# anoma/taiga

Measured on NVIDIA H100. Metric: partial-tx proofs/sec, higher is better.
Workload: dtype u32x8 (255-bit Montgomery integers, Pasta Fp/Fq)

## Files before the change

### taiga_b200/csrc/msm.cu

```cuda
#include <memory>
#include "common.cuh"
#include "kernels.cuh"

namespace tb {

constexpr int MSM_CHUNK_MAX = 64;
constexpr int MSM_SEG = 8;
constexpr int MSM_FIXED_C = 13;
constexpr uint32_t MSM_HEAVY_UNITS = 1024;

int msm_default_window(int n, bool fixed_tables) {
  if (fixed_tables) return MSM_FIXED_C;
  int lg = 0; while ((1 << (lg + 1)) <= n) ++lg;
  int c = lg - 4;
  if (c < 4) c = 4;
  if (c > 16) c = 16;
  return c;
}

__device__ __forceinline__ uint32_t window_bits(const uint32_t* s, int bit, int c) {
  int limb = bit >> 5, off = bit & 31;
  uint64_t v = s[limb];
  if (limb + 1 < 8) v |= (uint64_t)s[limb + 1] << 32;
  return (uint32_t)(v >> off) & ((1u << c) - 1);
// ... 193 lines not shown
    { const uint32_t* src = reinterpret_cast<const uint32_t*>(&acc); uint32_t* dst = reinterpret_cast<uint32_t*>(&o);
#pragma unroll
      for (int i = 0; i < 32; ++i) dst[i] = __shfl_down_sync(0xffffffffu, src[i], d, 16); }
    if ((int)l < d) acc.add(o);
  }
  if (live && l == 0) lines[line] = acc;
}
template <class B>
__global__ void __launch_bounds__(256) msm_weighted_kernel(const Xyzz<B>* __restrict__ lines, int s_log, int h_log, Xyzz<B>* __restrict__ out, Aff<B>* __restrict__ aff_out) {
  extern __shared__ uint4 mw_smem[];
  Xyzz<B>* sm = reinterpret_cast<Xyzz<B>*>(mw_smem);
  const int S = 1 << s_log, H = 1 << h_log, half = blockDim.x >> 1;
  const int part = threadIdx.x >= (unsigned)half, j = threadIdx.x - part * half, len = part ? H : S;
  const Xyzz<B>* src = lines + (size_t)blockIdx.x * (S + H) + (part ? S : 0);
  Xyzz<B>* v = sm + part * half;
  Xyzz<B> acc = j < len ? src[j] : Xyzz<B>::inf();
  v[j] = acc;
  __syncthreads();
  for (int d = 1; d < half; d <<= 1) {
    const bool act = j + d < len;
    Xyzz<B> o;
    if (act) o = v[j + d];
    __syncthreads();
    if (act) { acc.add(o); v[j] = acc; }
    __syncthreads();
  }
  if (part && j == 0) v[0] = Xyzz<B>::inf();
  __syncthreads();
  for (int d = half >> 1; d >= 1; d >>= 1) {
    if (j < d) { Xyzz<B> a = v[j]; a.add(v[j + d]); v[j] = a; }
    __syncthreads();
  }
  if (threadIdx.x == 0) {
    Xyzz<B> r = sm[half];
    for (int i = 0; i < s_log; ++i) r = r.dbl();
    r.add(sm[0]);
    out[blockIdx.x] = r;
    if (aff_out) aff_out[blockIdx.x] = r.to_affine();
  }
}

template <class B>
__global__ void __launch_bounds__(256) msm_window_kernel(const Xyzz<B>* __restrict__ seg_out, int nt, Xyzz<B>* __restrict__ win_out) {
  __shared__ Xyzz<B> sm[8];
  uint32_t g = blockIdx.x;
  Xyzz<B> acc = Xyzz<B>::inf();
  for (int t = threadIdx.x; t < nt; t += blockDim.x) acc.add(seg_out[(size_t)g * nt + t]);
  acc = block_reduce_pt(acc, sm);
  if (threadIdx.x == 0) win_out[g] = acc;
}

template <class B>
__global__ void msm_horner_kernel(const Xyzz<B>* __restrict__ win, int wsep, int c, int K, Xyzz<B>* __restrict__ out) {
  int k = blockIdx.x * blockDim.x + threadIdx.x;
  if (k >= K) return;
  Xyzz<B> acc = win[(size_t)k * wsep + wsep - 1];
  for (int w = wsep - 2; w >= 0; --w) {
    for (int i = 0; i < c; ++i) acc = acc.dbl();
    acc.add(win[(size_t)k * wsep + w]);
  }
  out[k] = acc;
}

template <class B, class S>
void msm_run(Ctx* ctx, const S* scalars, long long scalar_bstride, const Aff<B>* bases, long long base_bstride, int N, int K,
             const MsmConfig& cfg_in, Xyzz<B>* out) {
  TB_REQUIRE(N >= 1 && K >= 1 && K <= 65535, "MSM shape out of range");
  const bool table_mode = cfg_in.table_windows > 0;
  int c = cfg_in.c ? cfg_in.c : msm_default_window(N, table_mode);
  TB_REQUIRE(c >= 2 && c <= 20, "MSM window out of range");
  const int W = (256 + c - 1) / c;
  if (table_mode) TB_REQUIRE(cfg_in.table_windows >= W, "fixed-base table has too few windows");
  const int NB = 1 << (c - 1);
  const int wsep = table_mode ? 1 : W;
  const uint64_t nb_total64 = (uint64_t)K * wsep * NB;
  const int n_extra = table_mode ? cfg_in.n_extra : 0;
  const int table_stride = table_mode ? (cfg_in.table_stride ? cfg_in.table_stride : N) : 0;
  const uint64_t max_entries = (uint64_t)K * (N + n_extra) * W;
  TB_REQUIRE(nb_total64 < (1ull << 31) && max_entries < (1ull << 32) && (uint64_t)(N + 2) * (table_mode ? W : 1) < (1ull << 31), "MSM too large");
  const uint32_t nb_total = (uint32_t)nb_total64;
  cudaStream_t st = ctx->stream;

  DevBuf<Xyzz<B>> buckets(ctx, nb_total);
  ctx->work[PC_MSM_SORT] += 2.0 * (double)K * (N + n_extra);
  ctx->work[PC_MSM_REDUCE] += (double)K * wsep * NB * 30.0;
  std::unique_ptr<ProfScope> ps;
  if (msm_batch_applicable(N, K, cfg_in, c)) {
    msm_batch_buckets<B, S>(ctx, scalars, scalar_bstride, bases, N, K, c, W, table_stride, reinterpret_cast<const S*>(cfg_in.extra_scalars), n_extra, buckets.get());
    ctx->launches -= 6;
  } else {
    DevBuf<uint32_t> counts(ctx, nb_total), offs(ctx, nb_total + 1), cursor(ctx, nb_total), entries(ctx, max_entries);
    ps.reset(new ProfScope(ctx, PC_MSM_SORT));
    counts.zero();
    dim3 dg((N + n_extra + 255) / 256, K);
    const S* extras = reinterpret_cast<const S*>(cfg_in.extra_scalars);
    msm_digits_kernel<S, 0><<<dg, 256, 0, st>>>(scalars, scalar_bstride, N, c, W, NB, wsep, table_mode, table_stride, extras, n_extra, counts.get(), nullptr);
    TB_LAUNCH_CHECK();
    exclusive_scan_u32(ctx, counts.get(), offs.get(), nb_total);
    TB_CUDA(cudaMemcpyAsync(cursor.get(), offs.get(), nb_total * sizeof(uint32_t), cudaMemcpyDeviceToDevice, st));
    msm_digits_kernel<S, 1><<<dg, 256, 0, st>>>(scalars, scalar_bstride, N, c, W, NB, wsep, table_mode, table_stride, extras, n_extra, cursor.get(), entries.get());
    TB_LAUNCH_CHECK();

    uint32_t chunk_log = 3;
    { const uint64_t target_units = (uint64_t)tb_tune("TB_MSM_UNITS_PER_SM", 2048) * (uint64_t)ctx->sm_count;
      while ((1u << chunk_log) < (uint32_t)MSM_CHUNK_MAX && (max_entries >> chunk_log) > target_units) ++chunk_log; }
    const uint64_t max_units = nb_total64 + (max_entries >> chunk_log) + 1;
    const uint64_t max_heavy = (max_entries >> chunk_log) / MSM_HEAVY_UNITS + 1;
    uint32_t lpb_log = 0;
    { const uint64_t avg_units = ((max_entries >> chunk_log) + nb_total64 - 1) / nb_total64;
      const uint64_t warps_target = (uint64_t)tb_tune("TB_MSM_SUB_WARPS_PER_SM", 16) * (uint64_t)ctx->sm_count;
      while (lpb_log < 5 && ((nb_total64 << (lpb_log + 1)) >> 5) <= warps_target && (1ull << lpb_log) < avg_units) ++lpb_log; }
    const uint32_t sub_units = 4u << lpb_log;
    uint64_t max_mid = (max_entries >> chunk_log) / sub_units + 1;
    if (max_mid > nb_total64) max_mid = nb_total64;
    DevBuf<uint32_t> unit_count(ctx, nb_total), unit_off(ctx, nb_total + 1), mid(ctx, max_mid), heavy(ctx, max_heavy), n_lists(ctx, 2);
    n_lists.zero();
    msm_units_kernel<<<(nb_total + 255) / 256, 256, 0, st>>>(offs.get(), nb_total, chunk_log, sub_units, unit_count.get(), mid.get(), heavy.get(), n_lists.get());
    TB_LAUNCH_CHECK();
    exclusive_scan_u32(ctx, unit_count.get(), unit_off.get(), nb_total);
    DevBuf<Xyzz<B>> partial(ctx, max_units);
    ctx->work[PC_MSM_ACCUM] += 10.5 * (double)max_entries * 0.97;
    ps.reset(); ps.reset(new ProfScope(ctx, PC_MSM_ACCUM));
    { const unsigned ag = (unsigned)((max_units + 127) / 128);
      const int minb = tb_tune("TB_MSM_ACCUM_MINB", 4);
      if (minb >= 6) msm_accum_kernel<B, 6><<<ag, 128, 0, st>>>(bases, base_bstride, (uint32_t)wsep * NB, offs.get(), unit_off.get(), nb_total, 1u << chunk_log, entries.get(), partial.get());
      else if (minb == 5) msm_accum_kernel<B, 5><<<ag, 128, 0, st>>>(bases, base_bstride, (uint32_t)wsep * NB, offs.get(), unit_off.get(), nb_total, 1u << chunk_log, entries.get(), partial.get());
      else msm_accum_kernel<B, 4><<<ag, 128, 0, st>>>(bases, base_bstride, (uint32_t)wsep * NB, offs.get(), unit_off.get(), nb_total, 1u << chunk_log, entries.get(), partial.get()); }
    TB_LAUNCH_CHECK();
    ps.reset(); ps.reset(new ProfScope(ctx, PC_MSM_REDUCE));
    msm_combine_sub_kernel<B><<<(unsigned)((((uint64_t)nb_total << lpb_log) + 127) / 128), 128, 0, st>>>(unit_off.get(), partial.get(), nb_total, lpb_log,
                                                                                                        buckets.get());
    { uint64_t g = (max_mid + 7) / 8, cap = 4ull * (uint64_t)ctx->sm_count;
      msm_combine_kernel<B><<<(unsigned)(g < cap ? g : cap), 256, 0, st>>>(mid.get(), n_lists.get(), unit_off.get(), partial.get(), buckets.get()); }
    if ((max_entries >> chunk_log) > MSM_HEAVY_UNITS)
      msm_combine_heavy_kernel<B><<<(unsigned)(max_heavy < 296 ? max_heavy : 296), 256, 0, st>>>(heavy.get(), n_lists.get() + 1, unit_off.get(), partial.get(), buckets.get());
    TB_LAUNCH_CHECK();
    ps.reset();
  }
  ps.reset(new ProfScope(ctx, PC_MSM_REDUCE));

  const int seg_t = tb_tune("TB_MSM_SEG", MSM_SEG);
  const int seg = NB < seg_t ? NB : seg_t;
  const int nt = NB / seg;
  const uint32_t groups = (uint32_t)K * wsep;
  Aff<B>* const aff_out = reinterpret_cast<Aff<B>*>(cfg_in.affine_out);
  if (wsep == 1 && NB < 64) {
    int threads = ((nt + 31) / 32) * 32;
    msm_bucket_reduce_kernel<B><<<groups, threads, 0, st>>>(buckets.get(), NB, seg, nt, out, aff_out);
    TB_LAUNCH_CHECK();
    ctx->launches += 6;
    return;
  }
  if (wsep == 1) {
    const int lb = c - 1, s_log = (lb + 1) / 2, h_log = lb - s_log;
    const int nl = (1 << s_log) + (1 << h_log), threads = 2 << s_log;
    TB_REQUIRE(threads <= 256, "fixed-base window too wide for the weighted-sum kernel (c <= 15)");
    DevBuf<Xyzz<B>> lines(ctx, (size_t)groups * nl);
    msm_linesum_kernel<B><<<(unsigned)(((uint64_t)groups * nl * 16 + 127) / 128), 128, 0, st>>>(buckets.get(), NB, s_log, groups, lines.get());
    TB_LAUNCH_CHECK();
    const size_t smem = (size_t)threads * sizeof(Xyzz<B>);
    if (smem > 48 * 1024) {
      ctx->opt_in_smem(msm_weighted_kernel<B>, 128 * 1024);
    }
    msm_weighted_kernel<B><<<groups, threads, smem, st>>>(lines.get(), s_log, h_log, out, aff_out);
    TB_LAUNCH_CHECK();
    ctx->launches += 7;
    return;
  }
  DevBuf<Xyzz<B>> seg_out(ctx, (size_t)groups * nt), win(ctx, groups);
  msm_segsum_kernel<B><<<(groups * nt + 127) / 128, 128, 0, st>>>(buckets.get(), NB, seg, nt, groups, seg_out.get());
  TB_LAUNCH_CHECK();
  msm_window_kernel<B><<<groups, 256, 0, st>>>(seg_out.get(), nt, win.get());
  TB_LAUNCH_CHECK();
  msm_horner_kernel<B><<<(K + 31) / 32, 32, 0, st>>>(win.get(), wsep, c, K, out);
// ... 65 lines not shown
```

### taiga_b200/csrc/msm_batch.cu

```cuda
#define TB_NOINLINE_MUL 0
#include <cuda.h>
#include <algorithm>
#include <memory>
#include <type_traits>
#include "common.cuh"
#include "kernels.cuh"

namespace tb {

constexpr int BA_THREADS = 256;
constexpr int BA_M = 32;
constexpr int BA_PAIRS = BA_THREADS * BA_M;
constexpr int BA_MAX_NB = 4096;
constexpr int SORT_THREADS = 1024;
constexpr int SORT_TILE = 1024;
constexpr int SORT_BOX = 256;

__device__ __forceinline__ void block_scan_excl(uint32_t* v, int n, uint32_t* tmp) {
  const int T = blockDim.x, t = threadIdx.x, per = (n + T - 1) / T;
  const int b0 = t * per, b1 = min(n, b0 + per);
  uint32_t local = 0;
  for (int i = b0; i < b1; ++i) local += v[i];
  uint32_t incl = local;
  const int lane = t & 31, warp = t >> 5, nw = (T + 31) >> 5;
#pragma unroll
  for (int d = 1; d < 32; d <<= 1) { uint32_t o = __shfl_up_sync(0xffffffffu, incl, d); if (lane >= d) incl += o; }
  if (lane == 31) tmp[warp] = incl;
  __syncthreads();
  if (warp == 0) {
    uint32_t w = lane < nw ? tmp[lane] : 0u, wi = w;
#pragma unroll
    for (int d = 1; d < 32; d <<= 1) { uint32_t o = __shfl_up_sync(0xffffffffu, wi, d); if (lane >= d) wi += o; }
    if (lane < nw) tmp[lane] = wi - w;
    if (lane == nw - 1) v[n] = wi;
  }
  __syncthreads();
  uint32_t run = tmp[warp] + incl - local;
  for (int i = b0; i < b1; ++i) { uint32_t x = v[i]; v[i] = run; run += x; }
  __syncthreads();
}

__device__ __forceinline__ uint32_t smem_u32(const void* p) { return (uint32_t)__cvta_generic_to_shared(p); }
__device__ __forceinline__ void mbar_init(uint64_t* bar, uint32_t count) {
  asm volatile("mbarrier.init.shared::cta.b64 [%0], %1;" ::"r"(smem_u32(bar)), "r"(count) : "memory");
}
__device__ __forceinline__ void mbar_expect_tx(uint64_t* bar, uint32_t bytes) {
  asm volatile("mbarrier.arrive.expect_tx.shared::cta.b64 _, [%0], %1;" ::"r"(smem_u32(bar)), "r"(bytes) : "memory");
}
__device__ __forceinline__ void mbar_wait(uint64_t* bar, uint32_t parity) {
  uint32_t done = 0;
  for (uint32_t spin = 0; spin < (1u << 26); ++spin) {
    asm volatile("{ .reg .pred p; mbarrier.try_wait.parity.shared::cta.b64 p, [%1], %2; selp.u32 %0, 1, 0, p; }" : "=r"(done) : "r"(smem_u32(bar)), "r"(parity) : "memory");
    if (done) return;
  }
  __trap();
}
__device__ __forceinline__ void tma_load_tile(void* dst, const CUtensorMap* map, uint64_t* bar, int scalar0, int item) {
  asm volatile("cp.async.bulk.tensor.3d.shared::cluster.global.tile.mbarrier::complete_tx::bytes [%0], [%1, {%3, %4, %5}], [%2];"
               ::"r"(smem_u32(dst)), "l"(map), "r"(smem_u32(bar)), "r"(0), "r"(scalar0), "r"(item) : "memory");
}

template <class S, int CT>
__global__ void __launch_bounds__(SORT_THREADS) msm_sort_kernel(const __grid_constant__ CUtensorMap smap, const S* __restrict__ extras, int N, int n_extra, int c_rt, int W_rt,
                                                                 int NB, int table_stride, uint32_t* __restrict__ counts, uint32_t* __restrict__ entries, long long cap0,
                                                                 unsigned long long* __restrict__ total_entries) {
  const int c = CT ? CT : c_rt, W = CT ? (256 + CT - 1) / CT : W_rt;
  extern __shared__ __align__(128) uint8_t sort_smem[];
  S* tile = reinterpret_cast<S*>(sort_smem);
  uint64_t* bars = reinterpret_cast<uint64_t*>(sort_smem + 2 * SORT_TILE * sizeof(S));
  uint32_t* hist = reinterpret_cast<uint32_t*>(bars + 2);
  uint32_t* tmp = hist + NB + 1;
  const int k = blockIdx.x, t = threadIdx.x;
  const uint32_t half = 1u << (c - 1);
  const int ntiles = (N + SORT_TILE - 1) / SORT_TILE;
  if (t == 0) { mbar_init(&bars[0], 1); mbar_init(&bars[1], 1); asm volatile("fence.mbarrier_init.release.cluster;" ::: "memory"); }
  for (int b = t; b <= NB; b += SORT_THREADS) hist[b] = 0;
  __syncthreads();
  uint32_t* ent = entries + (long long)k * cap0;

  auto digits = [&](const S& sm, uint32_t idx, auto scatter_c) {
    constexpr bool scatter = decltype(scatter_c)::value;
    S s = sm.from_mont();
    if (s.is_zero()) return;
    uint32_t carry = 0;
#pragma unroll
    for (int w = 0; w < W; ++w) {
      const int bit = w * c, limb = bit >> 5, off = bit & 31;
      uint64_t v64 = s.l[limb];
      if (limb + 1 < 8) v64 |= (uint64_t)s.l[limb + 1] << 32;
      uint32_t v = ((uint32_t)(v64 >> off) & ((1u << c) - 1)) + carry, neg = 0;
      if (v > half) { v = (1u << c) - v; neg = 1; carry = 1; } else carry = 0;
      if (v) {
        if (scatter) { const uint32_t pos = atomicAdd(&hist[v - 1], 1u); ent[pos] = (uint32_t)(w * table_stride + idx) | (neg << 31); }
        else atomicAdd(&hist[v - 1], 1u);
      }
    }
  };
  auto issue = [&](int stage, int it) {
    const int s0 = it * SORT_TILE;
    int nbox = (N - s0 + SORT_BOX - 1) / SORT_BOX; if (nbox > SORT_TILE / SORT_BOX) nbox = SORT_TILE / SORT_BOX;
    mbar_expect_tx(&bars[stage], (uint32_t)(nbox * SORT_BOX * sizeof(S)));
    for (int j = 0; j < nbox; ++j) tma_load_tile(tile + stage * SORT_TILE + j * SORT_BOX, &smap, &bars[stage], s0 + j * SORT_BOX, k);
  };
  uint32_t phase[2] = {0, 0};
  for (int pass = 0; pass < 2; ++pass) {
    if (t == 0) issue(0, 0);
    for (int it = 0; it < ntiles; ++it) {
      const int st = it & 1;
      if (t == 0 && it + 1 < ntiles) issue(st ^ 1, it + 1);
      mbar_wait(&bars[st], phase[st]); phase[st] ^= 1;
      const int i = it * SORT_TILE + t;
      if (i < N) { if (pass) digits(tile[st * SORT_TILE + t], (uint32_t)i, std::true_type()); else digits(tile[st * SORT_TILE + t], (uint32_t)i, std::false_type()); }
      __syncthreads();
    }
    if (t < n_extra) { const S ex = ldg_fe(extras + (long long)k * n_extra + t); if (pass) digits(ex, (uint32_t)(N + t), std::true_type()); else digits(ex, (uint32_t)(N + t), std::false_type()); }
    __syncthreads();
    if (pass == 0) {
      for (int b = t; b < NB; b += SORT_THREADS) counts[(long long)k * NB + b] = hist[b];
      __syncthreads();
      block_scan_excl(hist, NB, tmp);
      if (t == 0) atomicAdd(total_entries, (unsigned long long)hist[NB]);
    }
  }
}

template <class F> __device__ __forceinline__ void sts_fe(uint4* lo, uint4* hi, int idx, const F& v) {
  lo[idx] = make_uint4(v.l[0], v.l[1], v.l[2], v.l[3]); hi[idx] = make_uint4(v.l[4], v.l[5], v.l[6], v.l[7]);
}
template <class F> __device__ __forceinline__ F lds_fe(const uint4* lo, const uint4* hi, int idx) {
  uint4 x = lo[idx], y = hi[idx]; F v;
  v.l[0] = x.x; v.l[1] = x.y; v.l[2] = x.z; v.l[3] = x.w; v.l[4] = y.x; v.l[5] = y.y; v.l[6] = y.z; v.l[7] = y.w; return v;
}

enum { PK_NONE = 0, PK_COPY1, PK_COPY2, PK_ADD, PK_DBL, PK_INF };

struct RoundOffsets {
  uint32_t* off_cur; uint32_t* off_nxt; uint32_t n_next;
  __device__ __forceinline__ void build(uint8_t* smem, const uint32_t* __restrict__ counts0, int NB, int round) {
    off_cur = reinterpret_cast<uint32_t*>(smem); off_nxt = off_cur + (NB + 4);
    uint32_t* tmp = off_nxt + (NB + 4);
    for (int b = threadIdx.x; b < NB; b += blockDim.x) {
      const uint32_t c0 = counts0[b], cr = (c0 + ((1u << round) - 1)) >> round;
      off_cur[b] = cr; off_nxt[b] = (cr + 1) >> 1;
    }
    __syncthreads();
    block_scan_excl(off_cur, NB, tmp);
    block_scan_excl(off_nxt, NB, tmp);
    n_next = off_nxt[NB];
  }
  __device__ __forceinline__ void locate(uint32_t q, int NB, uint32_t& in0, bool& two, int& hint) const {
    int lo = hint;
#pragma unroll 1
    for (int s = 0; s < 6 && off_nxt[lo + 1] <= q; ++s) ++lo;
    if (off_nxt[lo + 1] <= q) {
      int hi = NB;
      while (hi - lo > 1) { const int mid = (lo + hi) >> 1; if (off_nxt[mid] <= q) lo = mid; else hi = mid; }
    }
    hint = lo;
    in0 = off_cur[lo] + 2 * (q - off_nxt[lo]);
    two = in0 + 1 < off_cur[lo + 1];
  }
};
constexpr size_t ba_off_bytes(int NB) { return (size_t)(2 * (NB + 4) + 32) * 4; }

template <class B, bool FIRST> struct PairLoader {
  const uint32_t* entries; const Aff<B>* table; const Aff<B>* items;
  __device__ __forceinline__ Aff<B> point(uint32_t pos) const {
    if (FIRST) {
      const uint32_t e = __ldg(entries + pos);
      Aff<B> p = ldg_aff(table + (e & 0x7fffffffu));
      if (e >> 31) p.y = p.y.neg();
      return p;
    }
    return ldg_aff(items + pos);
  }
  __device__ __forceinline__ B x(uint32_t pos) const {
    if (FIRST) return ldg_fe(&table[__ldg(entries + pos) & 0x7fffffffu].x);
    return ldg_fe(&items[pos].x);
  }
};
template <class B> __device__ __forceinline__ int classify_pair(const Aff<B>& p1, const Aff<B>& p2, bool two, B& den) {
  if (!two || p2.is_inf()) return PK_COPY1;
  if (p1.is_inf()) return PK_COPY2;
  den = p2.x - p1.x;
  if (!den.is_zero()) return PK_ADD;
  if (p1.y == p2.y && !p1.y.is_zero()) { den = p1.y.dbl(); return PK_DBL; }
  return PK_INF;
}

__global__ void __launch_bounds__(BA_THREADS) msm_ba_count_kernel(const uint32_t* __restrict__ counts0, int NB, int R, uint32_t* __restrict__ n_items) {
  __shared__ uint32_t red[BA_THREADS / 32];
  const int k = blockIdx.x, t = threadIdx.x;
  for (int r = 0; r <= R; ++r) {
    uint32_t s = 0;
    for (int b = t; b < NB; b += BA_THREADS) s += (counts0[(long long)k * NB + b] + ((1u << r) - 1)) >> r;
    for (int d = 16; d >= 1; d >>= 1) s += __shfl_down_sync(0xffffffffu, s, d);
    if ((t & 31) == 0) red[t >> 5] = s;
    __syncthreads();
    if (t == 0) { uint32_t tot = 0; for (int w = 0; w < BA_THREADS / 32; ++w) tot += red[w]; n_items[(long long)k * (R + 1) + r] = tot; }
    __syncthreads();
  }
}

template <class B, bool FIRST, int M>
__global__ void __launch_bounds__(BA_THREADS) msm_ba_fwd_kernel(const uint32_t* __restrict__ counts0, int NB, int round, const uint32_t* __restrict__ entries,
// ... 41 lines not shown
template <class B>
__global__ void msm_ba_inv_kernel(B* __restrict__ tree, uint32_t n_trees) {
  const uint32_t i = blockIdx.x * blockDim.x + threadIdx.x;
  if (i >= n_trees) return;
  B* root = tree + (size_t)i * (2 * BA_THREADS) + 1;
  st_fe(root, ld_fe(root).inv());
}

template <class B, bool FIRST, int M, int MINB>
__global__ void __launch_bounds__(BA_THREADS, MINB) msm_ba_bwd_kernel(const uint32_t* __restrict__ counts0, int NB, int round, const uint32_t* __restrict__ entries,
                                                                 const Aff<B>* __restrict__ table, const Aff<B>* __restrict__ items_in, long long cap_in,
                                                                 Aff<B>* __restrict__ items_out, long long cap_out, const B* __restrict__ pre, const B* __restrict__ tree,
                                                                 const uint32_t* __restrict__ meta, const uint32_t* __restrict__ n_items, int R) {
  extern __shared__ __align__(16) uint8_t ba_smem[];
  const int k = blockIdx.y, t = threadIdx.x;
  const uint32_t Q0 = blockIdx.x * (M * BA_THREADS);
  const uint32_t n_next = n_items[(long long)k * (R + 1) + round + 1];
  if (Q0 >= n_next) return;
  B* nd = reinterpret_cast<B*>(ba_smem);
  { const B* tr = tree + ((long long)k * gridDim.x + blockIdx.x) * (2 * BA_THREADS);
    nd[t] = ld_fe(tr + t); nd[BA_THREADS + t] = ld_fe(tr + BA_THREADS + t); }
  __syncthreads();
  for (int w = 1; w < BA_THREADS; w <<= 1) {
    B child_inv;
    const int node = w + (t >> 1);
    if (t < 2 * w) child_inv = nd[node] * nd[2 * node + ((t & 1) ^ 1)];
    __syncthreads();
    if (t < 2 * w) nd[2 * node + (t & 1)] = child_inv;
    __syncthreads();
  }
  B inv_run = nd[BA_THREADS + t];
  PairLoader<B, FIRST> ld{entries + (FIRST ? (long long)k * cap_in : 0), table, items_in + (FIRST ? 0 : (long long)k * cap_in)};
  const B* pre_k = pre + (long long)k * cap_out;
  const uint32_t* meta_k = meta + (long long)k * cap_out;
  Aff<B>* out = items_out + (long long)k * cap_out;
  int last = M - 1;
  while (last >= 0 && Q0 + (uint32_t)last * BA_THREADS + t >= n_next) --last;
#pragma unroll 1
  for (int i = last; i >= 0; --i) {
    const uint32_t q = Q0 + (uint32_t)i * BA_THREADS + t;
    const uint32_t mt = __ldg(meta_k + q);
    const uint32_t in0 = mt & 0x7fffffffu; const bool two = mt >> 31;
    const Aff<B> p1 = ld.point(in0);
    Aff<B> p2 = p1;
    if (two) p2 = ld.point(in0 + 1);
    B den;
    const int kind = classify_pair(p1, p2, two, den);
    Aff<B> r;
    if (kind == PK_COPY1) r = p1;
    else if (kind == PK_COPY2) r = p2;
    else if (kind == PK_INF) r = Aff<B>::inf();
    else {
      const B dinv = inv_run * ldg_fe(pre_k + q);
      inv_run = inv_run * den;
      B num;
      if (kind == PK_ADD) num = p2.y - p1.y;
      else { const B x2 = p1.x.sqr(); num = x2.dbl() + x2; }
      const B lam = num * dinv;
      r.x = lam.sqr() - p1.x - p2.x;
      r.y = lam * (p1.x - r.x) - p1.y;
    }
    st_fe(&out[q].x, r.x); st_fe(&out[q].y, r.y);
  }
}

template <class B>
__global__ void __launch_bounds__(BA_THREADS) msm_ba_finish_kernel(const uint32_t* __restrict__ counts0, int NB, int round, const Aff<B>* __restrict__ items, long long cap,
                                                                    Xyzz<B>* __restrict__ buckets) {
  extern __shared__ __align__(16) uint8_t fin_smem[];
  uint32_t* off = reinterpret_cast<uint32_t*>(fin_smem);
  uint32_t* tmp = off + NB + 4;
  const int k = blockIdx.y, t = threadIdx.x;
  for (int b = t; b < NB; b += BA_THREADS) { uint32_t c0 = counts0[(long long)k * NB + b]; off[b] = (c0 + ((1u << round) - 1)) >> round; }
  __syncthreads();
  block_scan_excl(off, NB, tmp);
  const int b = blockIdx.x * BA_THREADS + t;
  if (b >= NB) return;
  Xyzz<B> acc = Xyzz<B>::inf();
  const Aff<B>* it = items + (long long)k * cap;
  for (uint32_t p = off[b]; p < off[b + 1]; ++p) acc.add_affine(ldg_aff(it + p));
  buckets[(long long)k * NB + b] = acc;
}

typedef CUresult (*EncodeTiledFn)(CUtensorMap*, CUtensorMapDataType, cuuint32_t, void*, const cuuint64_t*, const cuuint64_t*, const cuuint32_t*, const cuuint32_t*,
                                  CUtensorMapInterleave, CUtensorMapSwizzle, CUtensorMapL2promotion, CUtensorMapFloatOOBfill);
static EncodeTiledFn encode_tiled_fn() {
  static EncodeTiledFn fn = nullptr;
  if (!fn) {
    void* p = nullptr; cudaDriverEntryPointQueryResult qr;
    TB_CUDA(cudaGetDriverEntryPoint("cuTensorMapEncodeTiled", &p, cudaEnableDefault, &qr));
    if (qr != cudaDriverEntryPointSuccess || !p) throw CudaError("cuTensorMapEncodeTiled is not available from this driver");
    fn = reinterpret_cast<EncodeTiledFn>(p);
  }
  return fn;
}

template <class B, bool FIRST, int M, int MINB>
static void launch_round_t(Ctx* ctx, dim3 grid, size_t fwd_smem, size_t bwd_smem, const uint32_t* counts, int NB, int r, const uint32_t* entries, const Aff<B>* table, const Aff<B>* in,
                           long long cap_in, Aff<B>* out, long long cap_out, B* pre, B* tree, uint32_t* meta, const uint32_t* n_items, int R, uint32_t n_trees) {
  cudaStream_t st = ctx->stream;
  ctx->opt_in_smem(msm_ba_fwd_kernel<B, FIRST, M>, fwd_smem);
  ctx->opt_in_smem(msm_ba_bwd_kernel<B, FIRST, M, MINB>, bwd_smem);
  msm_ba_fwd_kernel<B, FIRST, M><<<grid, BA_THREADS, fwd_smem, st>>>(counts, NB, r, entries, table, in, cap_in, cap_out, pre, tree, meta, n_items, R);
  msm_ba_inv_kernel<B><<<(n_trees + 63) / 64, 64, 0, st>>>(tree, n_trees);
  msm_ba_bwd_kernel<B, FIRST, M, MINB><<<grid, BA_THREADS, bwd_smem, st>>>(counts, NB, r, entries, table, in, cap_in, out, cap_out, pre, tree, meta, n_items, R);
}
template <class B, typename... A> static void launch_round(Ctx* ctx, int M, int minb, bool first, A... a) {
#define TB_LR(MM, NN) (first ? launch_round_t<B, true, MM, NN>(ctx, a...) : launch_round_t<B, false, MM, NN>(ctx, a...))
  if (M == 8) { if (minb == 2) TB_LR(8, 2); else if (minb == 3) TB_LR(8, 3); else TB_LR(8, 4); }
  else if (M == 32) { if (minb == 2) TB_LR(32, 2); else if (minb == 3) TB_LR(32, 3); else TB_LR(32, 4); }
  else { if (minb == 2) TB_LR(16, 2); else if (minb == 3) TB_LR(16, 3); else TB_LR(16, 4); }
#undef TB_LR
}

bool msm_batch_applicable(int N, int K, const MsmConfig& cfg, int c) {
  if (cfg.table_windows <= 0 || (1 << (c - 1)) > BA_MAX_NB || c < 6) return false;
  const long long min_terms = tb_tune("TB_MSM_BA_MIN_TERMS", 1 << 21);
  return (long long)N * K >= min_terms;
}

template <class B, class S>
void msm_batch_buckets(Ctx* ctx, const S* scalars, long long sstride, const Aff<B>* table, int N, int K, int c, int W, int table_stride, const S* extras, int n_extra,
                       Xyzz<B>* buckets) {
  const int NB = 1 << (c - 1);
  cudaStream_t st = ctx->stream;
  TB_REQUIRE(((uintptr_t)scalars & 15) == 0 && (sstride * (long long)sizeof(S)) % 16 == 0, "scalar vectors must be 16-byte aligned for TMA");
  const long long cap0 = (long long)(N + n_extra) * W;
  std::vector<long long> cap(1, cap0);
  const int R = tb_tune("TB_MSM_BA_ROUNDS", 10);
  TB_REQUIRE(R >= 1 && R <= 20, "TB_MSM_BA_ROUNDS out of range");
  for (int r = 0; r < R; ++r) cap.push_back((cap.back() + NB + 1) / 2);
  const int Kc_max = tb_tune("TB_MSM_BA_CHUNK", ctx->sm_count);
  const int Kc = K < Kc_max ? K : Kc_max;
  DevBuf<uint32_t> counts(ctx, (size_t)Kc * NB), entries(ctx, (size_t)Kc * cap0);
  DevBuf<Aff<B>> itA(ctx, (size_t)Kc * cap[1]), itB(ctx, (size_t)Kc * (R > 1 ? cap[2] : 1));
  const size_t sort_smem = 2 * SORT_TILE * sizeof(S) + 16 + (size_t)(NB + 1 + 32) * 4 + 16;
  const size_t fwd_smem = std::max(ba_off_bytes(NB), (size_t)2 * BA_THREADS * sizeof(B));
  const size_t bwd_smem = (size_t)2 * BA_THREADS * sizeof(B);
  const size_t fin_smem = (size_t)(NB + 4 + 32) * 4;
  ctx->opt_in_smem(msm_sort_kernel<S, 13>, sort_smem);
  ctx->opt_in_smem(msm_sort_kernel<S, 0>, sort_smem);
  ctx->opt_in_smem(msm_ba_finish_kernel<B>, fin_smem);
  const int Mv = tb_tune("TB_MSM_BA_M", 32) >= 32 ? 32 : tb_tune("TB_MSM_BA_M", 32) <= 8 ? 8 : 16, minb = tb_tune("TB_MSM_BA_MINB", 3) <= 2 ? 2 : tb_tune("TB_MSM_BA_MINB", 3) >= 4 ? 4 : 3;
  const long long pairs_per_cta = (long long)Mv * BA_THREADS;
  const unsigned ctas1 = (unsigned)((cap[1] + pairs_per_cta - 1) / pairs_per_cta);
  DevBuf<B> pre(ctx, (size_t)Kc * cap[1]), tree(ctx, (size_t)Kc * ctas1 * 2 * BA_THREADS);
  DevBuf<uint32_t> meta(ctx, (size_t)Kc * cap[1]), n_items(ctx, (size_t)Kc * (R + 1));
  for (int k0 = 0; k0 < K; k0 += Kc) {
    const int kc = K - k0 < Kc ? K - k0 : Kc;
    { ProfScope ps(ctx, PC_MSM_SORT);
      CUtensorMap smap;
      const cuuint64_t dims[3] = {8, (cuuint64_t)N, (cuuint64_t)kc};
      const cuuint64_t strides[2] = {sizeof(S), (cuuint64_t)sstride * sizeof(S)};
      const cuuint32_t box[3] = {8, SORT_BOX, 1}, estr[3] = {1, 1, 1};
      CUresult cr = encode_tiled_fn()(&smap, CU_TENSOR_MAP_DATA_TYPE_UINT32, 3, const_cast<S*>(scalars + (long long)k0 * sstride), dims, strides, box, estr,
                                      CU_TENSOR_MAP_INTERLEAVE_NONE, CU_TENSOR_MAP_SWIZZLE_NONE, CU_TENSOR_MAP_L2_PROMOTION_L2_128B, CU_TENSOR_MAP_FLOAT_OOB_FILL_NONE);
      if (cr != CUDA_SUCCESS) throw CudaError("cuTensorMapEncodeTiled failed for the scalar tensor (" + std::to_string((int)cr) + ")");
      const S* ex = extras ? extras + (long long)k0 * n_extra : nullptr;
      if (c == 13) msm_sort_kernel<S, 13><<<kc, SORT_THREADS, sort_smem, st>>>(smap, ex, N, extras ? n_extra : 0, c, W, NB, table_stride, counts.get(), entries.get(), cap0, ctx->d_msm_adds);
      else msm_sort_kernel<S, 0><<<kc, SORT_THREADS, sort_smem, st>>>(smap, ex, N, extras ? n_extra : 0, c, W, NB, table_stride, counts.get(), entries.get(), cap0, ctx->d_msm_adds);
      TB_LAUNCH_CHECK(); ctx->launches++; }
    { ProfScope ps(ctx, PC_MSM_ACCUM);
      msm_ba_count_kernel<<<kc, BA_THREADS, 0, st>>>(counts.get(), NB, R, n_items.get());
      for (int r = 0; r < R; ++r) {
        const Aff<B>* in = (r & 1) ? itA.get() : itB.get();
        Aff<B>* out = (r & 1) ? itB.get() : itA.get();
        const unsigned gx = (unsigned)((cap[r + 1] + pairs_per_cta - 1) / pairs_per_cta);
        dim3 grid(gx, kc);
        const uint32_t n_trees = gx * (uint32_t)kc;
        launch_round<B>(ctx, Mv, minb, r == 0, grid, fwd_smem, bwd_smem, counts.get(), NB, r, entries.get(), table, in, r == 0 ? cap0 : cap[r], out, cap[r + 1], pre.get(), tree.get(),
                        meta.get(), n_items.get(), R, n_trees);
        TB_LAUNCH_CHECK(); ctx->launches += 3;
      }
      const Aff<B>* last = (R & 1) ? itA.get() : itB.get();
      msm_ba_finish_kernel<B><<<dim3((NB + BA_THREADS - 1) / BA_THREADS, kc), BA_THREADS, fin_smem, st>>>(counts.get(), NB, R, last, cap[R], buckets + (size_t)k0 * NB);
      TB_LAUNCH_CHECK(); ctx->launches++; }
  }
}

template void msm_batch_buckets<Fq, Fp>(Ctx*, const Fp*, long long, const Aff<Fq>*, int, int, int, int, int, const Fp*, int, Xyzz<Fq>*);
template void msm_batch_buckets<Fp, Fq>(Ctx*, const Fq*, long long, const Aff<Fp>*, int, int, int, int, int, const Fq*, int, Xyzz<Fp>*);

}
```

Before: 14.93.

## Replace per-MSM single-CTA TMA bucket sort with tiled digit/prefix/scatter kernels

The old sort used one 1024-thread CTA per MSM, streaming scalars through TMA twice (a count pass and a scatter pass), so parallelism was limited to K blocks. The new path splits the scalars into tiles spread over many CTAs. A digit kernel writes packed 16-bit signed digits and per-tile histograms, a prefix kernel scans the histograms across tiles, and a scatter kernel stages entries in shared memory, then writes them out in bucket order with warp-aggregated atomics. This adds an intermediate digit buffer, extra global traffic and two more launches, and entry order within a bucket now differs.

After: 15.50, median of 6. +3.8%, better.

```diff
diff --git a/taiga_b200/csrc/msm.cu b/taiga_b200/csrc/msm.cu
--- a/taiga_b200/csrc/msm.cu
+++ b/taiga_b200/csrc/msm.cu
@@ -299,14 +299,15 @@
   cudaStream_t st = ctx->stream;
 
   DevBuf<Xyzz<B>> buckets(ctx, nb_total);
-  ctx->work[PC_MSM_SORT] += 2.0 * (double)K * (N + n_extra);
   ctx->work[PC_MSM_REDUCE] += (double)K * wsep * NB * 30.0;
   std::unique_ptr<ProfScope> ps;
   if (msm_batch_applicable(N, K, cfg_in, c)) {
+    ctx->work[PC_MSM_SORT] += (double)K * (N + n_extra);
     msm_batch_buckets<B, S>(ctx, scalars, scalar_bstride, bases, N, K, c, W, table_stride, reinterpret_cast<const S*>(cfg_in.extra_scalars), n_extra, buckets.get());
     ctx->launches -= 6;
   } else {
     DevBuf<uint32_t> counts(ctx, nb_total), offs(ctx, nb_total + 1), cursor(ctx, nb_total), entries(ctx, max_entries);
+    ctx->work[PC_MSM_SORT] += 2.0 * (double)K * (N + n_extra);
     ps.reset(new ProfScope(ctx, PC_MSM_SORT));
     counts.zero();
     dim3 dg((N + n_extra + 255) / 256, K);
diff --git a/taiga_b200/csrc/msm_batch.cu b/taiga_b200/csrc/msm_batch.cu
--- a/taiga_b200/csrc/msm_batch.cu
+++ b/taiga_b200/csrc/msm_batch.cu
@@ -1,8 +1,6 @@
 #define TB_NOINLINE_MUL 0
-#include <cuda.h>
 #include <algorithm>
 #include <memory>
-#include <type_traits>
 #include "common.cuh"
 #include "kernels.cuh"
 
@@ -12,9 +10,12 @@
 constexpr int BA_M = 32;
 constexpr int BA_PAIRS = BA_THREADS * BA_M;
 constexpr int BA_MAX_NB = 4096;
-constexpr int SORT_THREADS = 1024;
-constexpr int SORT_TILE = 1024;
-constexpr int SORT_BOX = 256;
+constexpr int DIG_THREADS = 256;
+constexpr int PREFIX_THREADS = 256;
+constexpr int SCAT_THREADS = 1024;
+constexpr int TILE_ENTRIES = 20480;
+__host__ __device__ constexpr int tile_log(int W) { return W <= 20 ? 10 : W <= 40 ? 9 : 8; }
+__host__ __device__ constexpr int dig_stride(int W) { return (W + 3) & ~3; }
 
 __device__ __forceinline__ void block_scan_excl(uint32_t* v, int n, uint32_t* tmp) {
   const int T = blockDim.x, t = threadIdx.x, per = (n + T - 1) / T;
@@ -40,87 +41,147 @@
   __syncthreads();
 }
 
-__device__ __forceinline__ uint32_t smem_u32(const void* p) { return (uint32_t)__cvta_generic_to_shared(p); }
-__device__ __forceinline__ void mbar_init(uint64_t* bar, uint32_t count) {
-  asm volatile("mbarrier.init.shared::cta.b64 [%0], %1;" ::"r"(smem_u32(bar)), "r"(count) : "memory");
-}
-__device__ __forceinline__ void mbar_expect_tx(uint64_t* bar, uint32_t bytes) {
-  asm volatile("mbarrier.arrive.expect_tx.shared::cta.b64 _, [%0], %1;" ::"r"(smem_u32(bar)), "r"(bytes) : "memory");
-}
-__device__ __forceinline__ void mbar_wait(uint64_t* bar, uint32_t parity) {
-  uint32_t done = 0;
-  for (uint32_t spin = 0; spin < (1u << 26); ++spin) {
-    asm volatile("{ .reg .pred p; mbarrier.try_wait.parity.shared::cta.b64 p, [%1], %2; selp.u32 %0, 1, 0, p; }" : "=r"(done) : "r"(smem_u32(bar)), "r"(parity) : "memory");
-    if (done) return;
-  }
-  __trap();
-}
-__device__ __forceinline__ void tma_load_tile(void* dst, const CUtensorMap* map, uint64_t* bar, int scalar0, int item) {
-  asm volatile("cp.async.bulk.tensor.3d.shared::cluster.global.tile.mbarrier::complete_tx::bytes [%0], [%1, {%3, %4, %5}], [%2];"
-               ::"r"(smem_u32(dst)), "l"(map), "r"(smem_u32(bar)), "r"(0), "r"(scalar0), "r"(item) : "memory");
-}
+template <bool RET> __device__ __forceinline__ uint32_t bucket_add(uint32_t* ctr, uint32_t key) {
+  const uint32_t ones = __ballot_sync(0xffffffffu, key == 0);
+  uint32_t slot = 0;
+  if (ones) {
+    const uint32_t lane = threadIdx.x & 31, leader = __ffs(ones) - 1;
+    uint32_t old = 0;
+    if (lane == leader) {
+      if (RET) old = atomicAdd(ctr, (uint32_t)__popc(ones));
+      else atomicAdd(ctr, (uint32_t)__popc(ones));
+    }
+    if (RET) slot = __shfl_sync(0xffffffffu, old, leader) + __popc(ones & ((1u << lane) - 1));
+  }
+  if (key != 0 && key != ~0u) {
+    if (RET) slot = atomicAdd(&ctr[key], 1u);
+    else atomicAdd(&ctr[key], 1u);
+  }
+  return slot;
+}
+
 
 template <class S, int CT>
-__global__ void __launch_bounds__(SORT_THREADS) msm_sort_kernel(const __grid_constant__ CUtensorMap smap, const S* __restrict__ extras, int N, int n_extra, int c_rt, int W_rt,
-                                                                 int NB, int table_stride, uint32_t* __restrict__ counts, uint32_t* __restrict__ entries, long long cap0,
-                                                                 unsigned long long* __restrict__ total_entries) {
-  const int c = CT ? CT : c_rt, W = CT ? (256 + CT - 1) / CT : W_rt;
-  extern __shared__ __align__(128) uint8_t sort_smem[];
-  S* tile = reinterpret_cast<S*>(sort_smem);
-  uint64_t* bars = reinterpret_cast<uint64_t*>(sort_smem + 2 * SORT_TILE * sizeof(S));
-  uint32_t* hist = reinterpret_cast<uint32_t*>(bars + 2);
-  uint32_t* tmp = hist + NB + 1;
-  const int k = blockIdx.x, t = threadIdx.x;
-  const uint32_t half = 1u << (c - 1);
-  const int ntiles = (N + SORT_TILE - 1) / SORT_TILE;
-  if (t == 0) { mbar_init(&bars[0], 1); mbar_init(&bars[1], 1); asm volatile("fence.mbarrier_init.release.cluster;" ::: "memory"); }
-  for (int b = t; b <= NB; b += SORT_THREADS) hist[b] = 0;
-  __syncthreads();
-  uint32_t* ent = entries + (long long)k * cap0;
-
-  auto digits = [&](const S& sm, uint32_t idx, auto scatter_c) {
-    constexpr bool scatter = decltype(scatter_c)::value;
-    S s = sm.from_mont();
-    if (s.is_zero()) return;
-    uint32_t carry = 0;
+__global__ void __launch_bounds__(DIG_THREADS) msm_tile_digits_kernel(const S* __restrict__ scalars, long long sstride, const S* __restrict__ extras, int N,
+                                                                      int n_extra, int c_rt, int NB, uint16_t* __restrict__ dig, uint32_t* __restrict__ tcnt) {
+  const int c = CT ? CT : c_rt, W = (256 + c - 1) / c, WP = dig_stride(W), TS = 1 << tile_log(W);
+  extern __shared__ uint32_t hist[];
+  const int t = blockIdx.x, k = blockIdx.y, T = gridDim.x;
+  const uint32_t half = 1u << (c - 1), mask = (1u << c) - 1;
+  for (int b = threadIdx.x; b < NB; b += DIG_THREADS) hist[b] = 0;
+  __syncthreads();
+  for (int j = threadIdx.x; j < TS; j += DIG_THREADS) {
+    const int i = t * TS + j;
+    const bool live = i < N + n_extra;
+    S s = S::zero();
+    if (i < N) s = ldg_fe(scalars + (long long)k * sstride + i);
+    else if (live) s = ldg_fe(extras + (long long)k * n_extra + (i - N));
+    s = s.from_mont();
+    uint2* out = reinterpret_cast<uint2*>(dig + (((long long)k * T + t) * TS + j) * WP);
+    uint32_t carry = 0, lo = 0, hi = 0;
 #pragma unroll
     for (int w = 0; w < W; ++w) {
       const int bit = w * c, limb = bit >> 5, off = bit & 31;
       uint64_t v64 = s.l[limb];
       if (limb + 1 < 8) v64 |= (uint64_t)s.l[limb + 1] << 32;
-      uint32_t v = ((uint32_t)(v64 >> off) & ((1u << c) - 1)) + carry, neg = 0;
+      uint32_t v = ((uint32_t)(v64 >> off) & mask) + carry, neg = 0;
       if (v > half) { v = (1u << c) - v; neg = 1; carry = 1; } else carry = 0;
-      if (v) {
-        if (scatter) { const uint32_t pos = atomicAdd(&hist[v - 1], 1u); ent[pos] = (uint32_t)(w * table_stride + idx) | (neg << 31); }
-        else atomicAdd(&hist[v - 1], 1u);
+      bucket_add<false>(hist, v ? v - 1 : ~0u);
+      const uint32_t d = v ? v | neg << 15 : 0;
+      switch (w & 3) { case 0: lo = d; hi = 0; break; case 1: lo |= d << 16; break; case 2: hi = d; break; default: hi |= d << 16; }
+      if (live && ((w & 3) == 3 || w == W - 1)) out[w >> 2] = make_uint2(lo, hi);
+    }
+  }
+  __syncthreads();
+  uint32_t* row = tcnt + ((long long)k * T + t) * NB;
+  for (int b = threadIdx.x; b < NB; b += DIG_THREADS) row[b] = hist[b];
+}
+
+__global__ void __launch_bounds__(PREFIX_THREADS) msm_tile_prefix_kernel(uint32_t* __restrict__ tcnt, int T, int NB, uint32_t* __restrict__ counts,
+                                                                          unsigned long long* __restrict__ total_entries) {
+  __shared__ uint32_t red[PREFIX_THREADS / 32];
+  const int k = blockIdx.y, q = blockIdx.x * PREFIX_THREADS + threadIdx.x, NQ = NB / 4;
+  uint32_t tot = 0;
+  if (q < NQ) {
+    uint4* p = reinterpret_cast<uint4*>(tcnt + (long long)k * T * NB) + q;
+    uint4 run = make_uint4(0, 0, 0, 0);
+    for (int t0 = 0; t0 < T; t0 += 8) {
+      uint4 x[8];
+#pragma unroll
+      for (int u = 0; u < 8; ++u) if (t0 + u < T) x[u] = p[(long long)(t0 + u) * NQ];
+#pragma unroll
+      for (int u = 0; u < 8; ++u) if (t0 + u < T) {
+        p[(long long)(t0 + u) * NQ] = run;
+        run.x += x[u].x; run.y += x[u].y; run.z += x[u].z; run.w += x[u].w;
       }
     }
-  };
-  auto issue = [&](int stage, int it) {
-    const int s0 = it * SORT_TILE;
-    int nbox = (N - s0 + SORT_BOX - 1) / SORT_BOX; if (nbox > SORT_TILE / SORT_BOX) nbox = SORT_TILE / SORT_BOX;
-    mbar_expect_tx(&bars[stage], (uint32_t)(nbox * SORT_BOX * sizeof(S)));
-    for (int j = 0; j < nbox; ++j) tma_load_tile(tile + stage * SORT_TILE + j * SORT_BOX, &smap, &bars[stage], s0 + j * SORT_BOX, k);
-  };
-  uint32_t phase[2] = {0, 0};
-  for (int pass = 0; pass < 2; ++pass) {
-    if (t == 0) issue(0, 0);
-    for (int it = 0; it < ntiles; ++it) {
-      const int st = it & 1;
-      if (t == 0 && it + 1 < ntiles) issue(st ^ 1, it + 1);
-      mbar_wait(&bars[st], phase[st]); phase[st] ^= 1;
-      const int i = it * SORT_TILE + t;
-      if (i < N) { if (pass) digits(tile[st * SORT_TILE + t], (uint32_t)i, std::true_type()); else digits(tile[st * SORT_TILE + t], (uint32_t)i, std::false_type()); }
-      __syncthreads();
-    }
-    if (t < n_extra) { const S ex = ldg_fe(extras + (long long)k * n_extra + t); if (pass) digits(ex, (uint32_t)(N + t), std::true_type()); else digits(ex, (uint32_t)(N + t), std::false_type()); }
-    __syncthreads();
-    if (pass == 0) {
-      for (int b = t; b < NB; b += SORT_THREADS) counts[(long long)k * NB + b] = hist[b];
-      __syncthreads();
-      block_scan_excl(hist, NB, tmp);
-      if (t == 0) atomicAdd(total_entries, (unsigned long long)hist[NB]);
-    }
+    reinterpret_cast<uint4*>(counts + (long long)k * NB)[q] = run;
+    tot = run.x + run.y + run.z + run.w;
+  }
+  for (int d = 16; d >= 1; d >>= 1) tot += __shfl_down_sync(0xffffffffu, tot, d);
+  if ((threadIdx.x & 31) == 0) red[threadIdx.x >> 5] = tot;
+  __syncthreads();
+  if (threadIdx.x == 0) {
+    unsigned long long s = 0;
+    for (int w = 0; w < PREFIX_THREADS / 32; ++w) s += red[w];
+    atomicAdd(total_entries, s);
+  }
+}
+
+template <int CT>
+__global__ void __launch_bounds__(SCAT_THREADS, CT ? 2 : 1) msm_tile_scatter_kernel(const uint16_t* __restrict__ dig, const uint32_t* __restrict__ tcnt,
+                                                                            const uint32_t* __restrict__ counts, int n_terms, int c_rt, int NB, int table_stride,
+                                                                            uint32_t* __restrict__ entries, long long cap0) {
+  const int c = CT ? CT : c_rt, W = (256 + c - 1) / c, WP = dig_stride(W), tl = tile_log(W), TS = 1 << tl;
+  extern __shared__ uint32_t sc_smem[];
+  uint32_t* cur = sc_smem;
+  uint32_t* dst = cur + NB + 1;
+  uint32_t* tmp = dst + NB + 1;
+  uint32_t* stage = tmp + 32;
+  const int t = blockIdx.x, k = blockIdx.y, T = gridDim.x, tid = threadIdx.x;
+  const uint32_t* cnt_k = counts + (long long)k * NB;
+  const uint32_t* before = tcnt + ((long long)k * T + t) * NB;
+  const uint32_t* upto = t + 1 < T ? before + NB : cnt_k;
+  for (int b = tid; b < NB; b += SCAT_THREADS) { cur[b] = __ldg(upto + b) - __ldg(before + b); dst[b] = __ldg(cnt_k + b); }
+  __syncthreads();
+  block_scan_excl(cur, NB, tmp);
+  block_scan_excl(dst, NB, tmp);
+  const uint32_t n_ent = cur[NB];
+  for (int b = tid; b < NB; b += SCAT_THREADS) dst[b] += __ldg(before + b) - cur[b];
+  __syncthreads();
+  constexpr int JN = 1024 / SCAT_THREADS;
+  const uint16_t* dig_t = dig + ((long long)k * T + t) * TS * WP;
+  for (int q = 0; q < WP; q += 4) {
+    uint32_t key[JN][4], word[JN][4];
+#pragma unroll
+    for (int u = 0; u < JN; ++u) {
+      const int j = tid + u * SCAT_THREADS;
+      uint2 g = make_uint2(0, 0);
+      if (j < TS && t * TS + j < n_terms) g = __ldg(reinterpret_cast<const uint2*>(dig_t + (long long)j * WP + q));
+#pragma unroll
+      for (int r = 0; r < 4; ++r) {
+        const uint32_t d = ((r & 2) ? g.y : g.x) >> ((r & 1) * 16) & 0xffffu;
+        key[u][r] = (d & 0x7fffu) - 1;
+        word[u][r] = (d & 0x8000u) | (uint32_t)(q + r) << tl | (uint32_t)j;
+      }
+    }
+    uint32_t slot[JN][4];
+#pragma unroll
+    for (int u = 0; u < JN; ++u)
+#pragma unroll
+      for (int r = 0; r < 4; ++r) slot[u][r] = bucket_add<true>(cur, key[u][r]);
+#pragma unroll
+    for (int u = 0; u < JN; ++u)
+#pragma unroll
+      for (int r = 0; r < 4; ++r) if (key[u][r] != ~0u) stage[slot[u][r]] = key[u][r] << 16 | word[u][r];
+  }
+  __syncthreads();
+  uint32_t* ent = entries + (long long)k * cap0;
+  const uint32_t i0 = (uint32_t)(t * TS), wmask = (1u << (15 - tl)) - 1;
+#pragma unroll 4
+  for (uint32_t p = tid; p < n_ent; p += SCAT_THREADS) {
+    const uint32_t s = stage[p], w = (s >> tl) & wmask;
+    ent[dst[s >> 16] + p] = (w * (uint32_t)table_stride + i0 + (s & (TS - 1))) | (s & 0x8000u) << 16;
   }
 }
 
@@ -328,19 +389,6 @@
   buckets[(long long)k * NB + b] = acc;
 }
 
-typedef CUresult (*EncodeTiledFn)(CUtensorMap*, CUtensorMapDataType, cuuint32_t, void*, const cuuint64_t*, const cuuint64_t*, const cuuint32_t*, const cuuint32_t*,
-                                  CUtensorMapInterleave, CUtensorMapSwizzle, CUtensorMapL2promotion, CUtensorMapFloatOOBfill);
-static EncodeTiledFn encode_tiled_fn() {
-  static EncodeTiledFn fn = nullptr;
-  if (!fn) {
-    void* p = nullptr; cudaDriverEntryPointQueryResult qr;
-    TB_CUDA(cudaGetDriverEntryPoint("cuTensorMapEncodeTiled", &p, cudaEnableDefault, &qr));
-    if (qr != cudaDriverEntryPointSuccess || !p) throw CudaError("cuTensorMapEncodeTiled is not available from this driver");
-    fn = reinterpret_cast<EncodeTiledFn>(p);
-  }
-  return fn;
-}
-
 template <class B, bool FIRST, int M, int MINB>
 static void launch_round_t(Ctx* ctx, dim3 grid, size_t fwd_smem, size_t bwd_smem, const uint32_t* counts, int NB, int r, const uint32_t* entries, const Aff<B>* table, const Aff<B>* in,
                            long long cap_in, Aff<B>* out, long long cap_out, B* pre, B* tree, uint32_t* meta, const uint32_t* n_items, int R, uint32_t n_trees) {
@@ -370,7 +418,7 @@
                        Xyzz<B>* buckets) {
   const int NB = 1 << (c - 1);
   cudaStream_t st = ctx->stream;
-  TB_REQUIRE(((uintptr_t)scalars & 15) == 0 && (sstride * (long long)sizeof(S)) % 16 == 0, "scalar vectors must be 16-byte aligned for TMA");
+  TB_REQUIRE(((uintptr_t)scalars & 15) == 0 && (sstride * (long long)sizeof(S)) % 16 == 0, "scalar vectors must be 16-byte aligned");
   const long long cap0 = (long long)(N + n_extra) * W;
   std::vector<long long> cap(1, cap0);
   const int R = tb_tune("TB_MSM_BA_ROUNDS", 10);
@@ -380,12 +428,15 @@
   const int Kc = K < Kc_max ? K : Kc_max;
   DevBuf<uint32_t> counts(ctx, (size_t)Kc * NB), entries(ctx, (size_t)Kc * cap0);
   DevBuf<Aff<B>> itA(ctx, (size_t)Kc * cap[1]), itB(ctx, (size_t)Kc * (R > 1 ? cap[2] : 1));
-  const size_t sort_smem = 2 * SORT_TILE * sizeof(S) + 16 + (size_t)(NB + 1 + 32) * 4 + 16;
   const size_t fwd_smem = std::max(ba_off_bytes(NB), (size_t)2 * BA_THREADS * sizeof(B));
   const size_t bwd_smem = (size_t)2 * BA_THREADS * sizeof(B);
   const size_t fin_smem = (size_t)(NB + 4 + 32) * 4;
-  ctx->opt_in_smem(msm_sort_kernel<S, 13>, sort_smem);
-  ctx->opt_in_smem(msm_sort_kernel<S, 0>, sort_smem);
+  const int n_ex = extras ? n_extra : 0, TS = 1 << tile_log(W), T = (N + n_ex + TS - 1) / TS;
+  DevBuf<uint16_t> dig(ctx, (size_t)Kc * T * TS * dig_stride(W));
+  DevBuf<uint32_t> tcnt(ctx, (size_t)Kc * T * NB);
+  const size_t scat_smem = (size_t)(2 * (NB + 1) + 32 + TILE_ENTRIES) * 4;
+  ctx->opt_in_smem(msm_tile_scatter_kernel<13>, scat_smem);
+  ctx->opt_in_smem(msm_tile_scatter_kernel<0>, scat_smem);
   ctx->opt_in_smem(msm_ba_finish_kernel<B>, fin_smem);
   const int Mv = tb_tune("TB_MSM_BA_M", 32) >= 32 ? 32 : tb_tune("TB_MSM_BA_M", 32) <= 8 ? 8 : 16, minb = tb_tune("TB_MSM_BA_MINB", 3) <= 2 ? 2 : tb_tune("TB_MSM_BA_MINB", 3) >= 4 ? 4 : 3;
   const long long pairs_per_cta = (long long)Mv * BA_THREADS;
@@ -395,17 +446,17 @@
   for (int k0 = 0; k0 < K; k0 += Kc) {
     const int kc = K - k0 < Kc ? K - k0 : Kc;
     { ProfScope ps(ctx, PC_MSM_SORT);
-      CUtensorMap smap;
-      const cuuint64_t dims[3] = {8, (cuuint64_t)N, (cuuint64_t)kc};
-      const cuuint64_t strides[2] = {sizeof(S), (cuuint64_t)sstride * sizeof(S)};
-      const cuuint32_t box[3] = {8, SORT_BOX, 1}, estr[3] = {1, 1, 1};
-      CUresult cr = encode_tiled_fn()(&smap, CU_TENSOR_MAP_DATA_TYPE_UINT32, 3, const_cast<S*>(scalars + (long long)k0 * sstride), dims, strides, box, estr,
-                                      CU_TENSOR_MAP_INTERLEAVE_NONE, CU_TENSOR_MAP_SWIZZLE_NONE, CU_TENSOR_MAP_L2_PROMOTION_L2_128B, CU_TENSOR_MAP_FLOAT_OOB_FILL_NONE);
-      if (cr != CUDA_SUCCESS) throw CudaError("cuTensorMapEncodeTiled failed for the scalar tensor (" + std::to_string((int)cr) + ")");
-      const S* ex = extras ? extras + (long long)k0 * n_extra : nullptr;
-      if (c == 13) msm_sort_kernel<S, 13><<<kc, SORT_THREADS, sort_smem, st>>>(smap, ex, N, extras ? n_extra : 0, c, W, NB, table_stride, counts.get(), entries.get(), cap0, ctx->d_msm_adds);
-      else msm_sort_kernel<S, 0><<<kc, SORT_THREADS, sort_smem, st>>>(smap, ex, N, extras ? n_extra : 0, c, W, NB, table_stride, counts.get(), entries.get(), cap0, ctx->d_msm_adds);
-      TB_LAUNCH_CHECK(); ctx->launches++; }
+      const S* sc = scalars + (long long)k0 * sstride;
+      const S* ex = n_ex ? extras + (long long)k0 * n_extra : nullptr;
+      const dim3 tg(T, kc);
+      if (c == 13) msm_tile_digits_kernel<S, 13><<<tg, DIG_THREADS, NB * 4, st>>>(sc, sstride, ex, N, n_ex, c, NB, dig.get(), tcnt.get());
+      else msm_tile_digits_kernel<S, 0><<<tg, DIG_THREADS, NB * 4, st>>>(sc, sstride, ex, N, n_ex, c, NB, dig.get(), tcnt.get());
+      TB_LAUNCH_CHECK();
+      msm_tile_prefix_kernel<<<dim3((NB / 4 + PREFIX_THREADS - 1) / PREFIX_THREADS, kc), PREFIX_THREADS, 0, st>>>(tcnt.get(), T, NB, counts.get(), ctx->d_msm_adds);
+      TB_LAUNCH_CHECK();
+      if (c == 13) msm_tile_scatter_kernel<13><<<tg, SCAT_THREADS, scat_smem, st>>>(dig.get(), tcnt.get(), counts.get(), N + n_ex, c, NB, table_stride, entries.get(), cap0);
+      else msm_tile_scatter_kernel<0><<<tg, SCAT_THREADS, scat_smem, st>>>(dig.get(), tcnt.get(), counts.get(), N + n_ex, c, NB, table_stride, entries.get(), cap0);
+      TB_LAUNCH_CHECK(); ctx->launches += 3; }
     { ProfScope ps(ctx, PC_MSM_ACCUM);
       msm_ba_count_kernel<<<kc, BA_THREADS, 0, st>>>(counts.get(), NB, R, n_items.get());
       for (int r = 0; r < R; ++r) {
```
